# apachepinot/pinot

Hardware: AMD Instinct MI355X
Metric: rows scanned/sec, 1B-row segment filter+groupby (3 predicates, SUM/MAX GROUP BY g1) (higher is better)
Workload: dtype int64; 1 GPU; 1 segment(s) x 1000000000 rows, one per GPU; SELECT g1, SUM(m), MAX(m) FROM gpuBench WHERE c_inv1 IN (0,1,2,3) AND c_inv2 IN (0,1) AND r_int BETWEEN 250000 AND 749999 GROUP BY g1 ORDER BY g1 LIMIT 1000; query=cfg3, parallelism=segment-per-gpu x1, merge=none (1 segment), entries_scanned_in_filter=249990290

## Files before the change

### pinot_amd/csrc/pg_kernels_spec.hip

```cpp
#define PG_WAVES_PER_BLOCK 12
#include "pg_kernel_agg.h"

#define SPEC_LOADERS 4
#ifndef SPEC_TILES
#define SPEC_TILES 2
#endif
#ifndef SPEC_SETS
#define SPEC_SETS 2
#endif
#define SPEC_CONSUMERS 8
#define SPEC_OFF_LIN 0u
#define SPEC_OFF_RNG 256u
#define SPEC_OFF_VAL (256u + 2048u)
#define SPEC_OFF_G0 (256u + 2048u + 8192u)
extern "C" const int pg_spec_waves_per_block = PG_WAVES_PER_BLOCK;
extern "C" int pg_spec_stage_bytes(int bits0, int bits1) { return SPEC_TILES * (((int)SPEC_OFF_G0 + bits0 * 256 + 16 + (bits1 > 0 ? bits1 * 256 + 16 : 0) + 15) & ~15); }

DEVFN void spec_barrier() {
  __builtin_amdgcn_fence(__ATOMIC_RELEASE, "workgroup", "local");
  __builtin_amdgcn_s_barrier();
  __builtin_amdgcn_fence(__ATOMIC_ACQUIRE, "workgroup", "local");
}

template <typename T> DEVFN const GAS T* spec_sgpr_ptr(const void* ptr) {
  const uint64_t v = (uint64_t)ptr;
  const uint32_t lo = (uint32_t)__builtin_amdgcn_readfirstlane((int)(uint32_t)v), hi = (uint32_t)__builtin_amdgcn_readfirstlane((int)(uint32_t)(v >> 32));
  return (const GAS T*)(((uint64_t)hi << 32) | (uint64_t)lo);
}

template <int W> struct SpecCol;
template <> struct SpecCol<0> {};
template <> struct SpecCol<32> { u32x4 r[2]; };
template <> struct SpecCol<24> { u32x4 lo; u32x2 hi; };
template <> struct SpecCol<16> { u32x4 lo; };
template <> struct SpecCol<8> { u32x2 hi; };
constexpr uint32_t spec_img_tile_bytes(int W) { return (uint32_t)(PG_WAVE_DOCS / 8) * (uint32_t)W; }
template <int W> DEVFN void spec_load(SpecCol<W>& c, const uint8_t* base, int wt, int w, int lane) {
  if constexpr (W == 32) {
#pragma unroll
    for (int s = 0; s < 2; s++) {
      const uint8_t* row = base + (size_t)wt * (PG_WAVE_DOCS * 4) + (size_t)(4 * s + w) * 1024u;
      c.r[s] = ldnt((const GAS u32x4*)(spec_sgpr_ptr<uint8_t>(row) + (uint32_t)lane * 16u));
    }
  } else if constexpr (W != 0) {
    const uint8_t* tile = base + (size_t)wt * spec_img_tile_bytes(W);
    if constexpr (W >= 16) c.lo = ldnt((const GAS u32x4*)(spec_sgpr_ptr<uint8_t>(tile + (size_t)w * 1024u) + (uint32_t)lane * 16u));
    if constexpr (W != 16) c.hi = ldnt((const GAS u32x2*)(spec_sgpr_ptr<uint8_t>(tile + (W == 24 ? 4096u : 0u) + (size_t)w * 512u) + (uint32_t)lane * 8u));
  }
}
template <int W> DEVFN void spec_unpack(const SpecCol<W>& c, uint32_t (&a)[4], uint32_t (&b)[4]) {
  if constexpr (W == 32) {
    a[0] = bswap32(c.r[0].x); a[1] = bswap32(c.r[0].y); a[2] = bswap32(c.r[0].z); a[3] = bswap32(c.r[0].w);
    b[0] = bswap32(c.r[1].x); b[1] = bswap32(c.r[1].y); b[2] = bswap32(c.r[1].z); b[3] = bswap32(c.r[1].w);
  } else if constexpr (W == 24) {
    a[0] = __builtin_amdgcn_perm(c.hi.x, c.lo.x, 0x0c040100u); a[1] = __builtin_amdgcn_perm(c.hi.x, c.lo.x, 0x0c050302u);
    a[2] = __builtin_amdgcn_perm(c.hi.x, c.lo.y, 0x0c060100u); a[3] = __builtin_amdgcn_perm(c.hi.x, c.lo.y, 0x0c070302u);
    b[0] = __builtin_amdgcn_perm(c.hi.y, c.lo.z, 0x0c040100u); b[1] = __builtin_amdgcn_perm(c.hi.y, c.lo.z, 0x0c050302u);
    b[2] = __builtin_amdgcn_perm(c.hi.y, c.lo.w, 0x0c060100u); b[3] = __builtin_amdgcn_perm(c.hi.y, c.lo.w, 0x0c070302u);
  } else if constexpr (W == 16) {
    a[0] = c.lo.x & 0xFFFFu; a[1] = c.lo.x >> 16; a[2] = c.lo.y & 0xFFFFu; a[3] = c.lo.y >> 16;
    b[0] = c.lo.z & 0xFFFFu; b[1] = c.lo.z >> 16; b[2] = c.lo.w & 0xFFFFu; b[3] = c.lo.w >> 16;
  } else if constexpr (W == 8) {
#pragma unroll
    for (int e = 0; e < 4; e++) { a[e] = (c.hi.x >> (8 * e)) & 0xFFu; b[e] = (c.hi.y >> (8 * e)) & 0xFFu; }
  }
}
template <int SW, int VW> struct SpecTile {
  SpecCol<SW> scan;
  SpecCol<VW> val;
  u32x4 grp;
};
template <int SW, int VW> struct SpecStage { SpecTile<SW, VW> tile[SPEC_TILES]; uint32_t post[8]; uint32_t tail; };
template <int NG> struct SpecQuad {
  uint32_t lin, rng;
  u32x4 val;
  uint32_t win[NG][2];
};

template <int W> struct SpecWidth { static constexpr int value = W; };
template <int NG, bool HAS_INDEX, bool HAS_SCAN, bool HAS_TAIL = false, bool NARROW = false>
__device__ __forceinline__ void spec_body(const PgQueryPlan& p) {
  extern __shared__ __attribute__((aligned(16))) uint64_t smem[];
  __shared__ uint32_t s_stat[PG_MAX_STATS];
  const int t = threadIdx.x;
  const int lane = t & 63;
  const int wave = uniform(t >> 6);
  int64_t* lds_table = reinterpret_cast<int64_t*>(smem);
  if (t < PG_MAX_STATS) s_stat[t] = 0;
  const uint32_t real_slots = (uint32_t)p.n_groups * (uint32_t)p.replicas;
  const uint32_t table_slots = real_slots + 64u;
  for (int o = 0; o < p.n_ops; o++) {
    const int64_t ident = pg_acc_identity(p.ops[o].fn, p.ops[o].is_float);
    for (uint32_t i = t; i < table_slots; i += PG_BLOCK) lds_table[(size_t)o * table_slots + i] = ident;
  }
  const uint32_t bits0 = (uint32_t)p.gcols[0].bits, bits1 = NG > 1 ? (uint32_t)p.gcols[NG - 1].bits : 0u;
  const uint32_t off_g1 = SPEC_OFF_G0 + bits0 * 256u + 16u;
  const uint32_t tile_bytes = (off_g1 + (NG > 1 ? bits1 * 256u + 16u : 0u) + 15u) & ~15u;
  const uint32_t stage_bytes = tile_bytes * SPEC_TILES;
  uint8_t* stage0 = reinterpret_cast<uint8_t*>(smem) + (((size_t)p.n_ops * table_slots * 8u + 15u) & ~(size_t)15u);
  const CAS PgScanLeaf& L = cptr(p.scans)[HAS_SCAN ? p.fast_scan : 0];
  const int grid = (int)gridDim.x;
  const int n_mine = (int)blockIdx.x < p.n_wtiles ? (p.n_wtiles - (int)blockIdx.x + grid - 1) / grid : 0;
  const int n_stages = (n_mine + SPEC_TILES - 1) / SPEC_TILES;
  __syncthreads();

  if (wave < SPEC_LOADERS) {
    const int w = wave;
    const uint8_t* const xdata = p.srcs[p.pipe_src].data;
    const uint8_t* const simg = NARROW ? p.spec_simg : nullptr;
    const uint8_t* const vimg = NARROW ? p.spec_vimg : nullptr;
    const uint32_t img_slo = NARROW ? p.spec_slo : 0u, img_sspan = NARROW ? p.spec_sspan : 0u, img_vmin = NARROW ? (uint32_t)p.spec_vmin : 0u;
    const bool img_sempty = NARROW && p.spec_sempty != 0;
    const int ggi = (w >> 1) < NG ? (w >> 1) : 0;
    const uint8_t* const gdata = p.gcols[ggi].data;
    const uint32_t gbits = (uint32_t)p.gcols[ggi].bits;
    const uint32_t goff = (uint32_t)(w & 1) * 1024u + (uint32_t)lane * 16u;
    const uint32_t geff = (w >> 1) < NG && goff < gbits * 256u ? goff : 0u;
    const uint8_t* dense_ptr[8];
    int dense_group[8];
#pragma unroll
    for (int j = 0; j < 8; j++) { dense_ptr[j] = HAS_INDEX ? p.dense_ptr[j] : nullptr; dense_group[j] = HAS_INDEX ? p.dense_group[j] : 0; }
    const int dense_groups = p.dense_groups, dense_excl = p.dense_excl;
    const uint8_t* const pipe_tail = HAS_TAIL ? p.pipe_tail : nullptr;
    const int num_docs = p.num_docs;
    const bool scan_pushed = p.fast_scan_pushed != 0;
   auto loaders = [&](auto scan_w, auto val_w) __attribute__((always_inline)) {
    constexpr int SW = HAS_SCAN ? decltype(scan_w)::value : 0, VW = decltype(val_w)::value;
    const RangeI32 r32 = !HAS_SCAN ? RangeI32{0, 0u, false} : (SW == 32 ? make_range_i32(L.lo, L.hi) : RangeI32{(int32_t)img_slo, img_sspan, img_sempty});
    const uint8_t* sdata = !HAS_SCAN ? nullptr : (SW == 32 ? L.data : simg);
    const uint8_t* vdata = VW == 32 ? xdata : vimg;
    const uint32_t vmin = VW == 32 ? 0u : img_vmin;
    uint32_t ld_cand = 0;
    auto issue = [&](int sidx, SpecStage<SW, VW>& st) __attribute__((always_inline)) {
#pragma unroll
      for (int tt = 0; tt < SPEC_TILES; tt++) {
        const int i = sidx * SPEC_TILES + tt;
        const int wt = (int)blockIdx.x + (i < n_mine ? i : n_mine - 1) * grid;
        SpecTile<SW, VW>& tl = st.tile[tt];
        __builtin_amdgcn_sched_barrier(0);
        spec_load<SW>(tl.scan, sdata, wt, w, lane);
        spec_load<VW>(tl.val, vdata, wt, w, lane);
        __builtin_amdgcn_sched_barrier(0);
        {
          const uint8_t* base = gdata + (size_t)wt * (size_t)(PG_WAVE_DOCS / 8) * (size_t)gbits;
          tl.grp = ldnt((const GAS u32x4*)(spec_sgpr_ptr<uint8_t>(base) + geff));
        }
        __builtin_amdgcn_sched_barrier(0);
      }
      if (HAS_INDEX) {
        const int i = sidx * SPEC_TILES + (w % SPEC_TILES);
        const int wt = (int)blockIdx.x + (i < n_mine ? i : n_mine - 1) * grid;
#pragma unroll
        for (int j = 0; j < 8; j++) st.post[j] = *(const GAS uint32_t*)(spec_sgpr_ptr<uint8_t>(dense_ptr[j] + (size_t)wt * 256u) + (uint32_t)lane * 4u);
        __builtin_amdgcn_sched_barrier(0);
      }
      if (HAS_TAIL) {
        const int i = sidx * SPEC_TILES + (w % SPEC_TILES);
        const int wt = (int)blockIdx.x + (i < n_mine ? i : n_mine - 1) * grid;
        st.tail = *(const GAS uint32_t*)(spec_sgpr_ptr<uint8_t>(pipe_tail + (size_t)wt * 256u) + (uint32_t)lane * 4u);
        __builtin_amdgcn_sched_barrier(0);
      }
    };
    auto publish = [&](uint8_t* stage, const SpecStage<SW, VW>& st) __attribute__((always_inline)) {
#ifdef PG_SPEC_NO_PUBLISH
      {
        uint32_t acc = 0;
#pragma unroll
        for (int tt = 0; tt < SPEC_TILES; tt++) {
          uint32_t a[4] = {0u, 0u, 0u, 0u}, b[4] = {0u, 0u, 0u, 0u};
          spec_unpack<SW>(st.tile[tt].scan, a, b); acc += a[0] ^ b[3];
          spec_unpack<VW>(st.tile[tt].val, a, b); acc += a[0] ^ b[3];
          acc += st.tile[tt].grp.x;
        }
        if (acc == 0x12345678u) *reinterpret_cast<uint32_t*>(stage) = acc;
        return;
      }
#endif
#pragma unroll
      for (int tt = 0; tt < SPEC_TILES; tt++) {
        uint8_t* buf = stage + (uint32_t)tt * tile_bytes;
        const SpecTile<SW, VW>& tl = st.tile[tt];
        if (HAS_SCAN) {
          uint32_t q[2][4];
          spec_unpack<SW>(tl.scan, q[0], q[1]);
#pragma unroll
          for (int s = 0; s < 2; s++) {
            uint32_t m = (uint32_t)in_range_i32(r32, (int32_t)q[s][0]) | ((uint32_t)in_range_i32(r32, (int32_t)q[s][1]) << 1) |
                         ((uint32_t)in_range_i32(r32, (int32_t)q[s][2]) << 2) | ((uint32_t)in_range_i32(r32, (int32_t)q[s][3]) << 3);
            m = r32.empty ? 0u : m;
            *reinterpret_cast<uint32_t*>(buf + SPEC_OFF_RNG + (uint32_t)(4 * s + w) * 256u + (uint32_t)lane * 4u) = m;
          }
        }
        {
          uint32_t q[2][4];
          spec_unpack<VW>(tl.val, q[0], q[1]);
#pragma unroll
          for (int s = 0; s < 2; s++) {
            u32x4 v;
            v.x = q[s][0] + vmin; v.y = q[s][1] + vmin; v.z = q[s][2] + vmin; v.w = q[s][3] + vmin;
            *reinterpret_cast<u32x4*>(buf + SPEC_OFF_VAL + (uint32_t)(4 * s + w) * 1024u + (uint32_t)lane * 16u) = v;
          }
        }
        *reinterpret_cast<u32x4*>(buf + (ggi == 0 ? SPEC_OFF_G0 : off_g1) + geff) = tl.grp;
      }
    };
    auto publish_lin = [&](uint8_t* stage, const SpecStage<SW, VW>& st, int sidx) __attribute__((always_inline)) {
      if (w >= SPEC_TILES) return;
      const int i = sidx * SPEC_TILES + w;
      const int wt = (int)blockIdx.x + i * grid;
      const int64_t rem = i < n_mine ? (int64_t)num_docs - (int64_t)wt * PG_WAVE_DOCS : 0;
      const int32_t n_valid = rem >= PG_WAVE_DOCS ? PG_WAVE_DOCS : (rem > 0 ? (int32_t)rem : 0);
      uint32_t lin = valid_lin_mask(n_valid, lane);
      if (HAS_INDEX) {
        uint32_t grp[4] = {0u, 0u, 0u, 0u};
#pragma unroll
        for (int j = 0; j < 8; j++) {
          const int gj = dense_group[j];
#pragma unroll
          for (int k = 0; k < 4; k++) grp[k] |= gj == k ? st.post[j] : 0u;
        }
#pragma unroll
        for (int k = 0; k < 4; k++)
          if (k < dense_groups) lin &= ((dense_excl >> k) & 1) ? ~grp[k] : grp[k];
      }
      *reinterpret_cast<uint32_t*>(stage + (uint32_t)w * tile_bytes + SPEC_OFF_LIN + (uint32_t)lane * 4u) = HAS_TAIL ? lin & st.tail : lin;
      ld_cand += (uint32_t)__popc(lin);
    };
    constexpr int SETS = HAS_SCAN ? SPEC_SETS : 2 * SPEC_SETS;
    SpecStage<SW, VW> st[SETS];
    auto buf_of = [&](int sg) __attribute__((always_inline)) { return stage0 + (uint32_t)(sg & 1) * stage_bytes; };
    if (n_stages > 0) {
#pragma unroll
      for (int k = 0; k < SETS; k++) issue(k, st[k]);
    }
    int s = 0;
    for (; s + SETS - 1 < n_stages; s += SETS) {
#pragma unroll
      for (int k = 0; k < SETS; k++) {
        publish(buf_of(s + k), st[k]);
        publish_lin(buf_of(s + k), st[k], s + k);
        issue(s + k + SETS, st[k]);
        spec_barrier();
      }
    }
#pragma unroll
    for (int k = 0; k < SETS - 1; k++)
      if (s + k < n_stages) {
        publish(buf_of(s + k), st[k]);
        publish_lin(buf_of(s + k), st[k], s + k);
        spec_barrier();
      }
    const uint32_t csum = wave_sum_u32(ld_cand);
    if (HAS_SCAN && !scan_pushed && lane == 0 && csum) atomicAdd(&s_stat[L.stat_slot], csum);
   };
    if constexpr (!NARROW) {
      loaders(SpecWidth<32>{}, SpecWidth<32>{});
    } else {
      const int sb = uniform(p.spec_sbits), vb = uniform(p.spec_vbits);
      auto with_scan = [&](auto scan_w) __attribute__((always_inline)) {
        switch (vb) {
          case 8: loaders(scan_w, SpecWidth<8>{}); break;
          case 16: loaders(scan_w, SpecWidth<16>{}); break;
          case 24: loaders(scan_w, SpecWidth<24>{}); break;
          default: loaders(scan_w, SpecWidth<32>{}); break;
        }
      };
      switch (sb) {
        case 8: with_scan(SpecWidth<8>{}); break;
        case 16: with_scan(SpecWidth<16>{}); break;
        case 24: with_scan(SpecWidth<24>{}); break;
        default: with_scan(SpecWidth<32>{}); break;
      }
    }
  } else {
    const int c = wave - SPEC_LOADERS;
    const uint32_t R = (uint32_t)p.replicas;
    const uint32_t rep = (uint32_t)t & (R - 1u);
    const uint32_t stride = table_slots;
    const uint32_t trash_slot = real_slots + (uint32_t)lane;
    const uint32_t q = (uint32_t)c * 64u + (uint32_t)lane;
    const uint32_t nib = ((uint32_t)lane & 7u) * 4u;
    uint32_t my_matched = 0;
    const int n_ops = uniform(p.n_ops);
    uint64_t ops_code = 0;
    for (int o = 0; o < n_ops; o++) {
      const PgAccOp op = p.ops[uniform(o)];
      ops_code |= (uint64_t)(op.src < 0 ? 0u : (op.fn == PG_ACC_SUM ? 1u : (op.fn == PG_ACC_MIN ? 2u : 3u))) << (2 * o);
    }
    ops_code = ((uint64_t)(uint32_t)uniform((int)(uint32_t)(ops_code >> 32)) << 32) | (uint64_t)(uint32_t)uniform((int)(uint32_t)ops_code);
    const int has_out_words = uniform(p.out_words != nullptr ? 1 : 0);
    auto fetch = [&](const uint8_t* buf, SpecQuad<NG>& d) __attribute__((always_inline)) {
      d.lin = *reinterpret_cast<const uint32_t*>(buf + SPEC_OFF_LIN + (q >> 3) * 4u);
      d.rng = HAS_SCAN ? *reinterpret_cast<const uint32_t*>(buf + SPEC_OFF_RNG + q * 4u) : 0xFu;
      d.val = *reinterpret_cast<const u32x4*>(buf + SPEC_OFF_VAL + q * 16u);
#pragma unroll
      for (int gi = 0; gi < NG; gi++) {
        const uint32_t di = __umul24(4u * q, (uint32_t)p.gcols[gi].bits) >> 5;
        const uint32_t* win = reinterpret_cast<const uint32_t*>(buf + (gi == 0 ? SPEC_OFF_G0 : off_g1)) + di;
        d.win[gi][0] = win[0]; d.win[gi][1] = win[1];
      }
    };
    auto aggregate = [&](const SpecQuad<NG> (&d)[SPEC_TILES], int sidx) __attribute__((always_inline)) {
      constexpr int ND = 4 * SPEC_TILES;
      uint32_t slot[ND];
      int32_t v[ND];
#pragma unroll
      for (int tt = 0; tt < SPEC_TILES; tt++) {
        const int i = sidx * SPEC_TILES + tt;
        const uint32_t cand = (d[tt].lin >> nib) & 0xFu;
        const uint32_t m = d[tt].rng & cand;
        my_matched += (uint32_t)__popc(m);
        if (has_out_words && i < n_mine) {
          const int wt = (int)blockIdx.x + i * grid;
          const uint32_t word = or_reduce8(m << nib);
          if ((lane & 7) == 0) reinterpret_cast<uint32_t*>(p.out_words)[(int64_t)wt * 64 + (int64_t)(q >> 3)] = word;
        }
#ifndef PG_SPEC_NO_TABLE
#pragma unroll
        for (int e = 0; e < 4; e++) slot[4 * tt + e] = rep;
#pragma unroll
        for (int gi = 0; gi < NG; gi++) {
          const PgGroupCol& gc = p.gcols[gi];
          const uint32_t bits = (uint32_t)gc.bits, mask = (1u << gc.bits) - 1u;
          const uint32_t mult = (uint32_t)gc.mult * R;
          uint32_t dv[4];
          decode_packed_quad<true>(d[tt].win[gi], q, bits, mask, dv);
#pragma unroll
          for (int e = 0; e < 4; e++) slot[4 * tt + e] += __umul24(dv[e], mult);
        }
#pragma unroll
        for (int e = 0; e < 4; e++) slot[4 * tt + e] = ((m >> e) & 1u) ? slot[4 * tt + e] : trash_slot;
        v[4 * tt + 0] = (int32_t)d[tt].val.x; v[4 * tt + 1] = (int32_t)d[tt].val.y; v[4 * tt + 2] = (int32_t)d[tt].val.z; v[4 * tt + 3] = (int32_t)d[tt].val.w;
#endif
      }
#ifdef PG_SPEC_NO_TABLE
      return;
#endif
      for (int o = 0; o < n_ops; o++) {
        const uint32_t code = (uint32_t)(ops_code >> (2 * o)) & 3u;
        int64_t* base = lds_table + (size_t)o * stride;
        if (code == 0u) {
#pragma unroll
          for (int e = 0; e < ND; e++) atomicAdd(reinterpret_cast<unsigned long long*>(base + slot[e]), 1ULL);
        } else if (code == 1u) {
#pragma unroll
          for (int e = 0; e < ND; e++) atomicAdd(reinterpret_cast<unsigned long long*>(base + slot[e]), (unsigned long long)(int64_t)v[e]);
        } else if (code == 2u) {
#pragma unroll
          for (int e = 0; e < ND; e++) atomicMin(reinterpret_cast<long long*>(base + slot[e]), (long long)v[e]);
        } else {
#pragma unroll
          for (int e = 0; e < ND; e++) atomicMax(reinterpret_cast<long long*>(base + slot[e]), (long long)v[e]);
        }
      }
    };
    auto fetch_stage = [&](int sidx, SpecQuad<NG> (&d)[SPEC_TILES]) __attribute__((always_inline)) {
      const uint8_t* stage = stage0 + (uint32_t)(sidx & 1) * stage_bytes;
#pragma unroll
      for (int tt = 0; tt < SPEC_TILES; tt++) fetch(stage + (uint32_t)tt * tile_bytes, d[tt]);
    };
    auto aggregate_stage = [&](int sidx, const SpecQuad<NG> (&d)[SPEC_TILES]) __attribute__((always_inline)) {
#ifdef PG_SPEC_NO_CONSUME
      return;
#endif
#ifdef PG_SPEC_FETCH_ONLY
      {
        uint32_t acc = 0;
#pragma unroll
        for (int tt = 0; tt < SPEC_TILES; tt++) { acc += d[tt].lin ^ d[tt].rng ^ d[tt].val.x ^ d[tt].val.w; for (int gi = 0; gi < NG; gi++) acc += d[tt].win[gi][0] ^ d[tt].win[gi][1]; }
        if (acc == 0x12345678u) my_matched++;
        return;
      }
#endif
      aggregate(d, sidx);
    };
    SpecQuad<NG> da[SPEC_TILES], db[SPEC_TILES];
    if (n_stages > 0) {
      spec_barrier();
#ifndef PG_SPEC_NO_CONSUME
      fetch_stage(0, da);
#endif
    }
    for (int s = 0; s < n_stages; s += 2) {
      if (s + 1 < n_stages) {
        spec_barrier();
#ifndef PG_SPEC_NO_CONSUME
        fetch_stage(s + 1, db);
#endif
      }
      aggregate_stage(s, da);
      if (s + 1 < n_stages) {
        if (s + 2 < n_stages) {
          spec_barrier();
#ifndef PG_SPEC_NO_CONSUME
          fetch_stage(s + 2, da);
#endif
        }
        aggregate_stage(s + 1, db);
      }
    }
    const uint32_t wsum = wave_sum_u32(my_matched);
    if (lane == 0 && wsum) atomicAdd(&s_stat[0], wsum);
  }
  __syncthreads();
  if (t < PG_MAX_STATS && s_stat[t]) atomicAdd(&p.stats[t], (unsigned long long)s_stat[t]);
  {
    const int R = p.replicas, groups = p.n_groups;
    int64_t* out = p.partials + (int64_t)blockIdx.x * ((int64_t)p.n_ops * groups);
    for (int o = 0; o < p.n_ops; o++) {
      const int fn = p.ops[uniform(o)].fn;
      for (int gq = t; gq < groups; gq += PG_BLOCK) {
        const int64_t* src = lds_table + (size_t)o * table_slots + (size_t)gq * R;
        int64_t acc = src[0];
        if (fn == PG_ACC_COUNT || fn == PG_ACC_SUM) { for (int r = 1; r < R; r++) acc += src[r]; }
        else if (fn == PG_ACC_MIN) { for (int r = 1; r < R; r++) acc = src[r] < acc ? src[r] : acc; }
        else { for (int r = 1; r < R; r++) acc = src[r] > acc ? src[r] : acc; }
        out[(size_t)o * groups + gq] = acc;
      }
    }
  }
}
#define PG_SPEC_KERNEL(NAME, IDX, SCAN) \
  extern "C" __global__ void __launch_bounds__(PG_BLOCK) NAME(const PgQueryPlan p) { \
    if (p.n_group_cols == 1) spec_body<1, IDX, SCAN>(p); \
    else spec_body<2, IDX, SCAN>(p); \
  }
PG_SPEC_KERNEL(pg_spec_none, false, false)
PG_SPEC_KERNEL(pg_spec_scan, false, true)
PG_SPEC_KERNEL(pg_spec_index, true, false)
#undef PG_SPEC_KERNEL
extern "C" __global__ void __launch_bounds__(PG_BLOCK) pg_fast_i32range_s(const PgQueryPlan p) {
  if (p.n_group_cols == 1) spec_body<1, true, true, false, true>(p);
  else spec_body<2, true, true, false, true>(p);
}
extern "C" __global__ void __launch_bounds__(PG_BLOCK) pg_fast_i32range_st(const PgQueryPlan p) {
  if (p.n_group_cols == 1) spec_body<1, true, true, true, true>(p);
  else spec_body<2, true, true, true, true>(p);
}
```

Measured before the change: 829.6 billion rows/s.

## Strength-reduce loader addressing with pinned SGPR bases and streamlined index mask algebra

Loader waves now keep per-column base pointers pinned in scalar registers and advance them incrementally per stage, with lane offsets held in fixed VGPRs. This replaces the per-tile recomputation of tile indices, clamping and readfirstlane address building. The dense-index posting combine becomes a branchless AND/OR chain driven by precomputed per-posting masks, and the remaining-doc count is decremented instead of recomputed. The aim is to cut scalar and vector ALU work and register pressure in the producer waves, at the cost of subtler clamp and advance logic that could go wrong at tile boundaries.

```diff
diff --git a/pinot_amd/csrc/pg_kernels_spec.hip b/pinot_amd/csrc/pg_kernels_spec.hip
--- a/pinot_amd/csrc/pg_kernels_spec.hip
+++ b/pinot_amd/csrc/pg_kernels_spec.hip
@@ -22,11 +22,15 @@
   __builtin_amdgcn_fence(__ATOMIC_ACQUIRE, "workgroup", "local");
 }
 
-template <typename T> DEVFN const GAS T* spec_sgpr_ptr(const void* ptr) {
-  const uint64_t v = (uint64_t)ptr;
-  const uint32_t lo = (uint32_t)__builtin_amdgcn_readfirstlane((int)(uint32_t)v), hi = (uint32_t)__builtin_amdgcn_readfirstlane((int)(uint32_t)(v >> 32));
-  return (const GAS T*)(((uint64_t)hi << 32) | (uint64_t)lo);
-}
+DEVFN uint32_t spec_pin(uint32_t v) {
+  v = (uint32_t)__builtin_amdgcn_readfirstlane((int)v);
+  asm volatile("" : "+s"(v));
+  return v;
+}
+DEVFN uint64_t spec_pin64(uint64_t v) { return ((uint64_t)spec_pin((uint32_t)(v >> 32)) << 32) | (uint64_t)spec_pin((uint32_t)v); }
+DEVFN void spec_lane_off(uint32_t& v) { asm volatile("" : "+v"(v)); }
+template <typename T> DEVFN T spec_ld(uint64_t base, uint32_t& voff) { spec_lane_off(voff); return *(const GAS T*)((const GAS uint8_t*)base + voff); }
+template <typename T> DEVFN T spec_ldnt(uint64_t base, uint32_t& voff) { spec_lane_off(voff); return ldnt((const GAS T*)((const GAS uint8_t*)base + voff)); }
 
 template <int W> struct SpecCol;
 template <> struct SpecCol<0> {};
@@ -35,17 +39,15 @@
 template <> struct SpecCol<16> { u32x4 lo; };
 template <> struct SpecCol<8> { u32x2 hi; };
 constexpr uint32_t spec_img_tile_bytes(int W) { return (uint32_t)(PG_WAVE_DOCS / 8) * (uint32_t)W; }
-template <int W> DEVFN void spec_load(SpecCol<W>& c, const uint8_t* base, int wt, int w, int lane) {
+constexpr uint32_t spec_col_tile_bytes(int W) { return W == 32 ? (uint32_t)PG_WAVE_DOCS * 4u : spec_img_tile_bytes(W); }
+struct SpecLaneOff { uint32_t row16, row16b, row8, row8b; };
+template <int W> DEVFN void spec_load(SpecCol<W>& c, uint64_t tile, SpecLaneOff& o) {
   if constexpr (W == 32) {
-#pragma unroll
-    for (int s = 0; s < 2; s++) {
-      const uint8_t* row = base + (size_t)wt * (PG_WAVE_DOCS * 4) + (size_t)(4 * s + w) * 1024u;
-      c.r[s] = ldnt((const GAS u32x4*)(spec_sgpr_ptr<uint8_t>(row) + (uint32_t)lane * 16u));
-    }
+    c.r[0] = spec_ldnt<u32x4>(tile, o.row16);
+    c.r[1] = spec_ldnt<u32x4>(tile, o.row16b);
   } else if constexpr (W != 0) {
-    const uint8_t* tile = base + (size_t)wt * spec_img_tile_bytes(W);
-    if constexpr (W >= 16) c.lo = ldnt((const GAS u32x4*)(spec_sgpr_ptr<uint8_t>(tile + (size_t)w * 1024u) + (uint32_t)lane * 16u));
-    if constexpr (W != 16) c.hi = ldnt((const GAS u32x2*)(spec_sgpr_ptr<uint8_t>(tile + (W == 24 ? 4096u : 0u) + (size_t)w * 512u) + (uint32_t)lane * 8u));
+    if constexpr (W >= 16) c.lo = spec_ldnt<u32x4>(tile, o.row16);
+    if constexpr (W != 16) c.hi = spec_ldnt<u32x2>(tile, W == 24 ? o.row8b : o.row8);
   }
 }
 template <int W> DEVFN void spec_unpack(const SpecCol<W>& c, uint32_t (&a)[4], uint32_t (&b)[4]) {
@@ -116,13 +118,38 @@
     const uint32_t gbits = (uint32_t)p.gcols[ggi].bits;
     const uint32_t goff = (uint32_t)(w & 1) * 1024u + (uint32_t)lane * 16u;
     const uint32_t geff = (w >> 1) < NG && goff < gbits * 256u ? goff : 0u;
-    const uint8_t* dense_ptr[8];
-    int dense_group[8];
-#pragma unroll
-    for (int j = 0; j < 8; j++) { dense_ptr[j] = HAS_INDEX ? p.dense_ptr[j] : nullptr; dense_group[j] = HAS_INDEX ? p.dense_group[j] : 0; }
-    const int dense_groups = p.dense_groups, dense_excl = p.dense_excl;
-    const uint8_t* const pipe_tail = HAS_TAIL ? p.pipe_tail : nullptr;
-    const int num_docs = p.num_docs;
+    SpecLaneOff loff = {(uint32_t)w * 1024u + (uint32_t)lane * 16u, 4096u + (uint32_t)w * 1024u + (uint32_t)lane * 16u,
+                        (uint32_t)w * 512u + (uint32_t)lane * 8u, 4096u + (uint32_t)w * 512u + (uint32_t)lane * 8u};
+    uint32_t post_off = (uint32_t)lane * 4u, grp_off = geff;
+    const uint32_t bx = spec_pin(blockIdx.x), ugrid = spec_pin((uint32_t)grid);
+    const int last = (int)spec_pin((uint32_t)(n_mine - 1));
+    const int stages = (int)spec_pin((uint32_t)n_stages);
+    const uint64_t g_base0 = spec_pin64((uint64_t)gdata + (uint64_t)bx * (uint64_t)(gbits * (uint32_t)(PG_WAVE_DOCS / 8)));
+    const uint32_t step256 = spec_pin(ugrid * (uint32_t)(PG_WAVE_DOCS / 8)), ugbits = spec_pin(gbits);
+    uint32_t grp_nend[8], grp_x[8];
+    if (HAS_INDEX) {
+      const uint32_t excl = (uint32_t)p.dense_excl;
+      const int last_group = p.dense_groups - 1;
+#pragma unroll
+      for (int j = 0; j < 8; j++) {
+        const int gj = p.dense_group[j];
+        const bool end = j < 7 ? p.dense_group[j < 7 ? j + 1 : j] != gj : gj == last_group;
+        const uint32_t xj = (excl >> gj) & 1u;
+        grp_x[j] = 0u - xj;
+        grp_nend[j] = (end ? 1u ^ xj : 0u) - 1u;
+        if (HAS_SCAN) { spec_lane_off(grp_x[j]); spec_lane_off(grp_nend[j]); }
+        else { grp_x[j] = spec_pin(grp_x[j]); grp_nend[j] = spec_pin(grp_nend[j]); }
+      }
+    }
+    const int p_pos0 = (int)(w % SPEC_TILES) < last ? (int)(w % SPEC_TILES) : last;
+    const uint64_t p_first = ((uint64_t)bx + (uint64_t)(uint32_t)(p_pos0 < 0 ? 0 : p_pos0) * (uint64_t)ugrid) * 256u;
+    const int p_left0 = (int)spec_pin((uint32_t)(last - p_pos0));
+    uint64_t p_base0[8];
+#pragma unroll
+    for (int j = 0; j < 8; j++) p_base0[j] = HAS_INDEX ? spec_pin64((uint64_t)p.dense_ptr[j] + p_first) : 0u;
+    const uint64_t t_base0 = HAS_TAIL ? spec_pin64((uint64_t)p.pipe_tail + p_first) : 0u;
+    const int64_t l_first = (int64_t)p.num_docs - ((int64_t)bx + (int64_t)w * (int64_t)ugrid) * PG_WAVE_DOCS;
+    const int32_t l_rem0 = (int32_t)spec_pin((uint32_t)(int32_t)(l_first > 0 ? l_first : -1));
     const bool scan_pushed = p.fast_scan_pushed != 0;
    auto loaders = [&](auto scan_w, auto val_w) __attribute__((always_inline)) {
     constexpr int SW = HAS_SCAN ? decltype(scan_w)::value : 0, VW = decltype(val_w)::value;
@@ -131,34 +158,49 @@
     const uint8_t* vdata = VW == 32 ? xdata : vimg;
     const uint32_t vmin = VW == 32 ? 0u : img_vmin;
     uint32_t ld_cand = 0;
-    auto issue = [&](int sidx, SpecStage<SW, VW>& st) __attribute__((always_inline)) {
+    uint64_t s_base = HAS_SCAN ? spec_pin64((uint64_t)sdata + (uint64_t)bx * spec_col_tile_bytes(SW)) : 0u;
+    uint64_t v_base = spec_pin64((uint64_t)vdata + (uint64_t)bx * spec_col_tile_bytes(VW));
+    uint64_t g_base = g_base0;
+    int steps_left = last;
+    uint64_t p_base[8], t_base = t_base0;
+#pragma unroll
+    for (int j = 0; j < 8; j++) p_base[j] = p_base0[j];
+    int p_left = p_left0;
+    int32_t l_rem = l_rem0;
+    auto issue = [&](SpecStage<SW, VW>& st) __attribute__((always_inline)) {
 #pragma unroll
       for (int tt = 0; tt < SPEC_TILES; tt++) {
-        const int i = sidx * SPEC_TILES + tt;
-        const int wt = (int)blockIdx.x + (i < n_mine ? i : n_mine - 1) * grid;
         SpecTile<SW, VW>& tl = st.tile[tt];
         __builtin_amdgcn_sched_barrier(0);
-        spec_load<SW>(tl.scan, sdata, wt, w, lane);
-        spec_load<VW>(tl.val, vdata, wt, w, lane);
+        spec_load<SW>(tl.scan, s_base, loff);
+        spec_load<VW>(tl.val, v_base, loff);
         __builtin_amdgcn_sched_barrier(0);
-        {
-          const uint8_t* base = gdata + (size_t)wt * (size_t)(PG_WAVE_DOCS / 8) * (size_t)gbits;
-          tl.grp = ldnt((const GAS u32x4*)(spec_sgpr_ptr<uint8_t>(base) + geff));
-        }
+        tl.grp = spec_ldnt<u32x4>(g_base, grp_off);
         __builtin_amdgcn_sched_barrier(0);
+        const uint32_t more = (uint32_t)(steps_left < 1 ? steps_left : 1);
+        steps_left -= (int)more;
+        const uint32_t adv = step256 * more;
+        if (HAS_SCAN) s_base += adv * (spec_col_tile_bytes(SW) / 256u);
+        v_base += adv * (spec_col_tile_bytes(VW) / 256u);
+        g_base += adv * ugbits;
       }
       if (HAS_INDEX) {
-        const int i = sidx * SPEC_TILES + (w % SPEC_TILES);
-        const int wt = (int)blockIdx.x + (i < n_mine ? i : n_mine - 1) * grid;
-#pragma unroll
-        for (int j = 0; j < 8; j++) st.post[j] = *(const GAS uint32_t*)(spec_sgpr_ptr<uint8_t>(dense_ptr[j] + (size_t)wt * 256u) + (uint32_t)lane * 4u);
+#pragma unroll
+        for (int j = 0; j < 8; j++) st.post[j] = spec_ld<uint32_t>(p_base[j], post_off);
         __builtin_amdgcn_sched_barrier(0);
       }
       if (HAS_TAIL) {
-        const int i = sidx * SPEC_TILES + (w % SPEC_TILES);
-        const int wt = (int)blockIdx.x + (i < n_mine ? i : n_mine - 1) * grid;
-        st.tail = *(const GAS uint32_t*)(spec_sgpr_ptr<uint8_t>(pipe_tail + (size_t)wt * 256u) + (uint32_t)lane * 4u);
+        st.tail = spec_ld<uint32_t>(t_base, post_off);
         __builtin_amdgcn_sched_barrier(0);
+      }
+      if (HAS_INDEX || HAS_TAIL) {
+        const int take = p_left < SPEC_TILES ? p_left : SPEC_TILES;
+        p_left -= take;
+        const uint32_t d = (uint32_t)take * step256;
+#pragma unroll
+        for (int j = 0; j < 8; j++)
+          if (HAS_INDEX) p_base[j] += d;
+        if (HAS_TAIL) t_base += d;
       }
     };
     auto publish = [&](uint8_t* stage, const SpecStage<SW, VW>& st) __attribute__((always_inline)) {
@@ -204,50 +246,56 @@
         *reinterpret_cast<u32x4*>(buf + (ggi == 0 ? SPEC_OFF_G0 : off_g1) + geff) = tl.grp;
       }
     };
-    auto publish_lin = [&](uint8_t* stage, const SpecStage<SW, VW>& st, int sidx) __attribute__((always_inline)) {
+    auto publish_lin = [&](uint8_t* stage, const SpecStage<SW, VW>& st) __attribute__((always_inline)) {
       if (w >= SPEC_TILES) return;
-      const int i = sidx * SPEC_TILES + w;
-      const int wt = (int)blockIdx.x + i * grid;
-      const int64_t rem = i < n_mine ? (int64_t)num_docs - (int64_t)wt * PG_WAVE_DOCS : 0;
-      const int32_t n_valid = rem >= PG_WAVE_DOCS ? PG_WAVE_DOCS : (rem > 0 ? (int32_t)rem : 0);
+      const int32_t rem = l_rem;
+      l_rem -= (int32_t)(step256 * (uint32_t)(SPEC_TILES * 8));
+      const int32_t n_valid = rem >= PG_WAVE_DOCS ? PG_WAVE_DOCS : (rem > 0 ? rem : 0);
       uint32_t lin = valid_lin_mask(n_valid, lane);
+#ifdef PG_SPEC_NO_INDEX_ALGEBRA
       if (HAS_INDEX) {
-        uint32_t grp[4] = {0u, 0u, 0u, 0u};
+        uint32_t acc = 0;
+#pragma unroll
+        for (int j = 0; j < 8; j++) acc ^= st.post[j];
+        lin = acc == 0x12345678u ? 0u : ~0u;
+      }
+#else
+      if (HAS_INDEX) {
+        uint32_t acc = 0u;
 #pragma unroll
         for (int j = 0; j < 8; j++) {
-          const int gj = dense_group[j];
-#pragma unroll
-          for (int k = 0; k < 4; k++) grp[k] |= gj == k ? st.post[j] : 0u;
-        }
-#pragma unroll
-        for (int k = 0; k < 4; k++)
-          if (k < dense_groups) lin &= ((dense_excl >> k) & 1) ? ~grp[k] : grp[k];
-      }
+          lin &= ~(st.post[j] & grp_x[j]);
+          acc |= st.post[j] & ~grp_x[j];
+          lin &= acc | grp_nend[j];
+          acc &= grp_nend[j];
+        }
+      }
+#endif
       *reinterpret_cast<uint32_t*>(stage + (uint32_t)w * tile_bytes + SPEC_OFF_LIN + (uint32_t)lane * 4u) = HAS_TAIL ? lin & st.tail : lin;
       ld_cand += (uint32_t)__popc(lin);
     };
     constexpr int SETS = HAS_SCAN ? SPEC_SETS : 2 * SPEC_SETS;
     SpecStage<SW, VW> st[SETS];
     auto buf_of = [&](int sg) __attribute__((always_inline)) { return stage0 + (uint32_t)(sg & 1) * stage_bytes; };
-    if (n_stages > 0) {
-#pragma unroll
-      for (int k = 0; k < SETS; k++) issue(k, st[k]);
+    if (stages > 0) {
+#pragma unroll
+      for (int k = 0; k < SETS; k++) issue(st[k]);
     }
     int s = 0;
-    for (; s + SETS - 1 < n_stages; s += SETS) {
+    for (; s + SETS - 1 < stages; s += SETS) {
 #pragma unroll
       for (int k = 0; k < SETS; k++) {
         publish(buf_of(s + k), st[k]);
-        publish_lin(buf_of(s + k), st[k], s + k);
-        issue(s + k + SETS, st[k]);
+        publish_lin(buf_of(s + k), st[k]);
+        issue(st[k]);
         spec_barrier();
       }
     }
 #pragma unroll
     for (int k = 0; k < SETS - 1; k++)
-      if (s + k < n_stages) {
+      if (s + k < stages) {
         publish(buf_of(s + k), st[k]);
-        publish_lin(buf_of(s + k), st[k], s + k);
+        publish_lin(buf_of(s + k), st[k]);
         spec_barrier();
       }
     const uint32_t csum = wave_sum_u32(ld_cand);
```

After: 827.9 billion rows/s. No clear change (-0.2%).
